# shichaoy/cube_slam

Hardware: AMD Instinct MI355X
Metric: frames/sec front-end (ORB extract + LSD+LBD lines + cuboid: Canny+DT+sweep+score+select) @640x480 (higher is better)
Workload: dtype f64

## Files before the change

cube_slam_amd/csrc/orb.hip:

```cpp
#include "common.h"
#include "orb_quadtree.h"

#include <cfloat>
#include <chrono>
#include <cmath>
#include <omp.h>

namespace {

constexpr int MAXL = 16;
constexpr int HALF_PATCH = 15, PATCH = 31, EDGE_T = 19, MINB = EDGE_T - 3;
constexpr int TW = 64, TH = 16;
constexpr int BLUR_ROWS = 64;

struct Lvl {
    int w, h;
    long off;
    int nCols, nRows, wCell, hCell, maxBX, maxBY;
    int cell_off;
    int tab_x, tab_y;
    float scale; int patch;
};
struct Pyr {
    int nlevels, cells_per_frame, ini_th, min_th;
    long frame_stride;
    int umax[HALF_PATCH + 1];
    int gk[7];
    int tile_off[MAXL + 1], blur_off[MAXL + 1];
    Lvl l[MAXL];
};

__constant__ int c_ring[16][2] = {{0, 3}, {1, 3}, {2, 2}, {3, 1}, {3, 0}, {3, -1}, {2, -2}, {1, -3}, {0, -3}, {-1, -3}, {-2, -2}, {-3, -1}, {-3, 0}, {-3, 1}, {-2, 2}, {-1, 3}};
__device__ const int d_pattern[1024] = {
#include "orb_pattern.inc"
};

#ifndef ORB_RS_ROWS
#define ORB_RS_ROWS 8
#endif
constexpr int RS_ROWS = ORB_RS_ROWS;
__global__ void __launch_bounds__(256) orb_resize(Pyr P, int level, uint8_t *__restrict__ pyr, const int *__restrict__ xofs, const short *__restrict__ ialpha, const int *__restrict__ yofs, const short *__restrict__ ibeta) {
    const Lvl &D = P.l[level], &S = P.l[level - 1];
    const int dx = (blockIdx.x * 64 + (threadIdx.x & 63)) * 4, dy0 = (blockIdx.y * 4 + __builtin_amdgcn_readfirstlane(threadIdx.x >> 6)) * RS_ROWS;
    if (dx >= D.w || dy0 >= D.h) return;
    uint8_t *base = pyr + (long)blockIdx.z * P.frame_stride;
    const uint8_t *src = base + S.off;
    const int nrow = min(RS_ROWS, D.h - dy0);
    int sx[4], a0[4], a1[4];
#pragma unroll
    for (int c = 0; c < 4; c++) {
        const int x = min(dx + c, D.w - 1);
        const int aa = reinterpret_cast<const int *>(ialpha)[D.tab_x + x];
        sx[c] = xofs[D.tab_x + x]; a0[c] = (short)(aa & 0xffff); a1[c] = aa >> 16;
    }
    const bool fast = dx + 3 < D.w && sx[3] - sx[0] <= 4 && sx[0] + 7 < S.w;
    if (fast) {
        uint32_t lo0[RS_ROWS], hi0[RS_ROWS], lo1[RS_ROWS], hi1[RS_ROWS]; int b0[RS_ROWS], b1[RS_ROWS];
#pragma unroll
        for (int r = 0; r < RS_ROWS; r++) {
            const int dy = min(dy0 + r, D.h - 1);
            const int sy = yofs[D.tab_y + dy], sy1 = min(sy + 1, S.h - 1);
            const int bb = reinterpret_cast<const int *>(ibeta)[D.tab_y + dy];
            b0[r] = (short)(bb & 0xffff); b1[r] = bb >> 16;
            const uint8_t *row0 = src + (long)sy * S.w + sx[0], *row1 = src + (long)sy1 * S.w + sx[0];
            lo0[r] = load_u32_unaligned(row0); hi0[r] = load_u32_unaligned(row0 + 4);
            lo1[r] = load_u32_unaligned(row1); hi1[r] = load_u32_unaligned(row1 + 4);
        }
        typedef unsigned short rs_v2u16 __attribute__((ext_vector_type(2)));
        uint32_t sel[4]; rs_v2u16 ap[4];
#pragma unroll
        for (int c = 0; c < 4; c++) { sel[c] = 0x0c010c00u + (uint32_t)(sx[c] - sx[0]) * 0x00010001u; ap[c] = __builtin_bit_cast(rs_v2u16, (uint32_t)a0[c] | ((uint32_t)a1[c] << 16)); }
#pragma unroll
        for (int r = 0; r < RS_ROWS; r++) {
            if (r >= nrow) break;
            uint32_t packed = 0;
#pragma unroll
            for (int c = 0; c < 4; c++) {
                const uint32_t r0 = __builtin_amdgcn_udot2(__builtin_bit_cast(rs_v2u16, __builtin_amdgcn_perm(hi0[r], lo0[r], sel[c])), ap[c], 0u, false);
                const uint32_t r1 = __builtin_amdgcn_udot2(__builtin_bit_cast(rs_v2u16, __builtin_amdgcn_perm(hi1[r], lo1[r], sel[c])), ap[c], 0u, false);
                const uint32_t v = ((__umul24((uint32_t)b0[r], r0 >> 4) >> 16) + (__umul24((uint32_t)b1[r], r1 >> 4) >> 16) + 2u) >> 2;
                packed |= (v & 255u) << (8 * c);
            }
            *reinterpret_cast<cs_u32_unaligned *>(base + D.off + (long)(dy0 + r) * D.w + dx) = packed;
        }
        return;
    }
    for (int r = 0; r < nrow; r++) {
        const int dy = dy0 + r, sy = yofs[D.tab_y + dy], sy1 = min(sy + 1, S.h - 1);
        const int b0 = ibeta[(D.tab_y + dy) * 2], b1 = ibeta[(D.tab_y + dy) * 2 + 1];
        const uint8_t *row0 = src + (long)sy * S.w, *row1 = src + (long)sy1 * S.w;
        for (int c = 0; c < 4 && dx + c < D.w; c++) {
            const int sxc = sx[c], sx1 = min(sxc + 1, S.w - 1);
            const int r0 = row0[sxc] * a0[c] + row0[sx1] * a1[c];
            const int r1 = row1[sxc] * a0[c] + row1[sx1] * a1[c];
            base[D.off + (long)dy * D.w + dx + c] = (uint8_t)((((b0 * (r0 >> 4)) >> 16) + ((b1 * (r1 >> 4)) >> 16) + 2) >> 2);
        }
    }
}

__global__ void __launch_bounds__(256) orb_fast_score(Pyr P, const uint8_t *pyr, uint8_t *smap) {
    int lvq = 0;
    while (lvq + 1 < P.nlevels && (int)blockIdx.x >= P.tile_off[lvq + 1]) lvq++;
    const int lv_u = __builtin_amdgcn_readfirstlane(lvq), tile = (int)blockIdx.x - P.tile_off[lv_u];
    const Lvl &L = P.l[lv_u];
    const int tiles_x = (L.w + TW - 1) / TW;
    const int tx0 = (tile % tiles_x) * TW, ty0 = (tile / tiles_x) * TH;
    __shared__ uint32_t g32[TH + 6][(TW + 8) / 4];
    __shared__ unsigned short s_list[TW * TH];
    __shared__ int s_n;
    uint8_t (*g)[TW + 8] = reinterpret_cast<uint8_t (*)[TW + 8]>(g32);
    const int tq = min(P.ini_th, P.min_th);
    const uint8_t *img = pyr + (long)blockIdx.z * P.frame_stride + L.off;
    if (threadIdx.x == 0) s_n = 0;
    for (int i = threadIdx.x; i < (TH + 6) * ((TW + 8) / 4); i += 256) {
        const int ly = i / ((TW + 8) / 4), k4 = i % ((TW + 8) / 4);
        const int X = tx0 + 4 * k4 - 3, Y = ty0 + ly - 3;
        uint32_t v = 0;
        if (Y >= 0 && Y < L.h) {
            const uint8_t *row = img + (long)Y * L.w;
            if (X >= 0 && X + 3 < L.w) v = load_u32_unaligned(row + X);
            else
                for (int c = 0; c < 4; c++) if (X + c >= 0 && X + c < L.w) v |= (uint32_t)row[X + c] << (8 * c);
        }
        g32[ly][k4] = v;
    }
    __syncthreads();
    const int lx = threadIdx.x & 63, wv = __builtin_amdgcn_readfirstlane((int)(threadIdx.x >> 6));
    static_assert(TH == 16, "four rows per wave");
    unsigned long long cm[4];
    const int x = tx0 + lx;
    const unsigned long long lt = (1ull << lx) - 1;
#pragma unroll
    for (int r = 0; r < 4; r++) {
        const int ly = wv + 4 * r, y = ty0 + ly;
        const int v = g[ly + 3][lx + 3];
        const int d0 = v - (int)g[ly + 6][lx + 3], d4 = v - (int)g[ly + 3][lx + 6], d8 = v - (int)g[ly][lx + 3], d12 = v - (int)g[ly + 3][lx];
        const int dark = max(max(min(d0, d4), min(d4, d8)), max(min(d8, d12), min(d12, d0)));
        const int bright = min(min(max(d0, d4), max(d4, d8)), min(max(d8, d12), max(d12, d0)));
        const bool inb = (unsigned)(x - 3) < (unsigned)(L.w - 6) & (unsigned)(y - 3) < (unsigned)(L.h - 6);
        const bool cand = inb & ((dark > tq) | (bright < -tq));
        if (!cand && x < L.w && y < L.h) smap[(long)blockIdx.z * P.frame_stride + L.off + (long)y * L.w + x] = 0;
        cm[r] = __ballot(cand);
    }
    const int c0 = __popcll(cm[0]), c1 = __popcll(cm[1]), c2 = __popcll(cm[2]), c3 = __popcll(cm[3]);
    if (c0 + c1 + c2 + c3) {
        int base = 0;
        if (lx == 0) base = atomicAdd(&s_n, c0 + c1 + c2 + c3);
        base = __builtin_amdgcn_readfirstlane(base);
        const int off[4] = {base, base + c0, base + c0 + c1, base + c0 + c1 + c2};
#pragma unroll
        for (int r = 0; r < 4; r++)
            if ((cm[r] >> lx) & 1ull) s_list[off[r] + __popcll(cm[r] & lt)] = (unsigned short)((wv + 4 * r) << 8 | lx);
    }
    __syncthreads();
    const int n = s_n;
    for (int i = threadIdx.x; i < n; i += 256) {
        const int ly = s_list[i] >> 8, px = s_list[i] & 255;
        const int v = g[ly + 3][px + 3];
        typedef short v2s __attribute__((ext_vector_type(2)));
        auto swp = [](v2s a) -> v2s { return __builtin_shufflevector(a, a, 1, 0); };
        v2s Pk[8];
#pragma unroll
        for (int k = 0; k < 8; k++) {
            const int ra = g[ly + 3 + c_ring[k][1]][px + 3 + c_ring[k][0]], rb = g[ly + 3 + c_ring[k + 8][1]][px + 3 + c_ring[k + 8][0]];
            v2s r; r.x = (short)(v - ra); r.y = (short)(v - rb);
            Pk[k] = r;
        }
        auto at = [&](const v2s (&X)[8], int k) -> v2s { k &= 15; return k < 8 ? X[k] : swp(X[k - 8]); };
        v2s lo2[8], hi2[8], lo4[8], hi4[8];
#pragma unroll
        for (int k = 0; k < 8; k++) { lo2[k] = __builtin_elementwise_min(Pk[k], at(Pk, k + 1)); hi2[k] = __builtin_elementwise_max(Pk[k], at(Pk, k + 1)); }
#pragma unroll
        for (int k = 0; k < 8; k++) { lo4[k] = __builtin_elementwise_min(lo2[k], at(lo2, k + 2)); hi4[k] = __builtin_elementwise_max(hi2[k], at(hi2, k + 2)); }
        v2s sdp = {-1000, -1000}, sbp = {1000, 1000};
#pragma unroll
        for (int k = 0; k < 8; k++) {
            const v2s lo9 = __builtin_elementwise_min(__builtin_elementwise_min(lo4[k], at(lo4, k + 4)), swp(Pk[k]));
            const v2s hi9 = __builtin_elementwise_max(__builtin_elementwise_max(hi4[k], at(hi4, k + 4)), swp(Pk[k]));
// ... 590 lines not shown
                            }
                            dead[id >> 5] |= 1u << (id & 31);
                        }
                        { int jn = 0; for (int q = 0; q < 4; q++) if (c[q] > 0) { if (c[q] > 1) { if (lane == 0) vn[nvn] = ((unsigned long long)c[q] << 32) | (unsigned)(nn + jn); nvn++; } jn++; } }
                        nn += kk; nfront += kk; cur += kk - 1;
                        __threadfence_block();
                        if (cur >= N) break;
                    }
                    if (cur >= N || cur == ps) fin = true;
                    { unsigned long long *t = vk; vk = vn; vn = t; }
                    nvk = nvn;
                }
                int o = 0;
                if (!ovf) {
                    for (int k0 = nfront - 1; k0 >= 0; k0 -= 64) {
                        const int k = k0 - lane;
                        int id = -1; bool al = false;
                        if (k >= 0) { id = front[k]; al = !((dead[id >> 5] >> (id & 31)) & 1u); }
                        const unsigned long long mm = __ballot(al);
                        if (al) nlist[o + __popcll(mm & ((1ull << lane) - 1))] = (short)id;
                        o += __popcll(mm);
                    }
                    for (int i0 = 0; i0 < n_list; i0 += 64) {
                        const int i = i0 + lane;
                        int id = -1; bool al = false;
                        if (i < n_list) { id = list[i]; al = !((dead[id >> 5] >> (id & 31)) & 1u); }
                        const unsigned long long mm = __ballot(al);
                        if (al) nlist[o + __popcll(mm & ((1ull << lane) - 1))] = (short)id;
                        o += __popcll(mm);
                    }
                }
                if (lane == 0) { s_i[1] = o; s_i[2] = ovf ? 1 : 0; }
            }
            __threadfence_block();
            __syncthreads();
            if (s_i[2]) { overflow = true; break; }
            n_list = s_i[1];
            { short *t = list; list = nlist; nlist = t; }
            finish = true;
        }
    }
    if (overflow) { if (tid == 0) { *status = 1; slot_cnt[fl] = 0; } return; }
    for (int i = tid; i < n_list; i += 256) {
        const int4 nd = nodes[list[i]];
        int best = perm[nd.z];
        float mxr = K[best * 3 + 2];
        for (int p = nd.z + 1; p < nd.w; p++) { const int idx = perm[p]; const float rr = K[idx * 3 + 2]; if (rr > mxr) { best = idx; mxr = rr; } }
        out[i] = SelKP{K[best * 3] + L.minX, K[best * 3 + 1] + L.minY, K[best * 3 + 2], lv, f};
    }
    if (tid == 0) slot_cnt[fl] = n_list;
}
__global__ void __launch_bounds__(256) orb_compact_sel(QtParams Q, const SelKP *slots, const int *slot_cnt, const int *sel_base, SelKP *sel) {
    const int lv = blockIdx.x, f = blockIdx.y, fl = f * Q.nlevels + lv;
    const SelKP *src = slots + (long)f * Q.slots_per_frame + Q.l[lv].slot_off;
    const int n = slot_cnt[fl], b = sel_base[fl];
    for (int i = threadIdx.x; i < n; i += 256) sel[b + i] = src[i];
}

static int qt_half_span(int lo, int hi, int cell, int n_cells, int extent) {
    int s = 0;
    for (int j = 0; j < n_cells; j++) {
        const int a = std::max(lo, 3 + j * cell), b = std::min(hi, std::min(3 + (j + 1) * cell, extent - 3));
        if (b > a) s += (b - a + 1) / 2;
    }
    return s;
}
static long qt_first_split_child_bound(const Lvl &L) {
    const int fw = L.maxBX - MINB, fh = L.maxBY - MINB;
    if (L.nCols < 1 || L.nRows < 1) return 0;
    const int nIni = (int)std::round(static_cast<float>(fw) / fh);
    if (nIni < 1 || nIni > 4) return 0;
    const float hX = static_cast<float>(fw) / nIni;
    const int my = (int)std::ceil(static_cast<float>(fh) / 2);
    const long rows = std::max(qt_half_span(0, my, L.hCell, L.nRows, fh), qt_half_span(my, fh, L.hCell, L.nRows, fh));
    long cols = 0;
    for (int b = 0; b < nIni; b++) {
        const int x0 = (int)(hX * static_cast<float>(b)), x1 = (int)(hX * static_cast<float>(b + 1)), mx = x0 + (int)std::ceil(static_cast<float>(x1 - x0) / 2);
        cols = std::max<long>(cols, qt_half_span(std::max(x0 - 1, 0), mx, L.wCell, L.nCols, fw));
        cols = std::max<long>(cols, qt_half_span(mx, b == nIni - 1 ? fw : x1 + 1, L.wCell, L.nCols, fw));
    }
    return cols * rows;
}

}

struct cs_orb {
    int nfeatures = 0, nlevels = 0, W = 0, H = 0, max_frames = 0, n_frames = 0;
    float scaleFactor = 0;
    std::vector<float> mvScaleFactor, mvInvScaleFactor, mvLevelSigma2, mvInvLevelSigma2;
    std::vector<int> mnFeaturesPerLevel;
    Pyr P{};
    int max_tiles = 0, max_blur_blocks = 0;
    long cand_cap = 0, cand_alloc = 0;
    uint8_t *d_pyr = nullptr, *d_smap = nullptr, *d_blur = nullptr;
    unsigned long long *d_cell_mask = nullptr;
    int *d_xofs = nullptr, *d_yofs = nullptr, *d_cell_count = nullptr, *d_cell_base = nullptr, *d_level_total = nullptr, *d_level_base = nullptr;
    short *d_ialpha = nullptr, *d_ibeta = nullptr;
    float *d_cand = nullptr, *d_angle = nullptr;
    SelKP *d_sel = nullptr;
    QtParams Q{}; bool gpu_quadtree = false; size_t qt_lds = 0;
    int *d_qperm = nullptr, *d_qtmp = nullptr, *d_slot_cnt = nullptr, *d_sel_base = nullptr, *d_qstatus = nullptr; int4 *d_qnodes = nullptr; SelKP *d_slots = nullptr;
    std::vector<int> sel_base;
    bool cand_valid = false;
    cs_keypoint *d_kps = nullptr;
    unsigned long long *d_desc = nullptr;
    long sel_cap = 0;
    std::vector<int> level_base;
    std::vector<cs_orb_host::Cand> cand;
    std::vector<SelKP> sel;
    std::vector<int> frame_first;
};

int cs_orb_device_frame(const cs_orb *e, int frame, const cs_keypoint **d_kps, const unsigned long long **d_desc, int *n) {
    if (!e || frame < 0 || frame >= e->n_frames || (int)e->frame_first.size() <= frame + 1) return CS_ERR_BAD_ARG;
    const int b0 = e->frame_first[frame];
    *d_kps = e->d_kps + b0; *d_desc = e->d_desc + (size_t)b0 * 4; *n = e->frame_first[frame + 1] - b0;
    return CS_OK;
}

int cs_orb_device_pyramid(const cs_orb *e, cs_orb_pyramid_view *out) {
    static_assert(CS_ORB_MAX_LEVELS == MAXL, "cs_orb_pyramid_view holds every level");
    if (!e || !out) return CS_ERR_BAD_ARG;
    out->d_pyr = e->d_pyr; out->frame_stride = e->P.frame_stride; out->nlevels = e->nlevels; out->n_frames = e->n_frames; out->W = e->W; out->H = e->H;
    out->scale_factor = e->scaleFactor;
    for (int l = 0; l < e->nlevels; l++) {
        out->off[l] = e->P.l[l].off; out->w[l] = e->P.l[l].w; out->h[l] = e->P.l[l].h;
        out->scale[l] = e->mvScaleFactor[l]; out->inv_scale[l] = e->mvInvScaleFactor[l];
    }
    return CS_OK;
}

extern "C" {

void cs_orb_destroy(cs_ctx *ctx, cs_orb *e) {
    if (!e) return;
    if (ctx) { hipSetDevice(ctx->device); hipStreamSynchronize(ctx->stream); }
    void *ptrs[] = {e->d_cell_mask, e->d_pyr, e->d_smap, e->d_blur, e->d_xofs, e->d_yofs, e->d_cell_count, e->d_cell_base, e->d_level_total, e->d_level_base,
                    e->d_ialpha, e->d_ibeta, e->d_cand, e->d_angle, e->d_sel, e->d_kps, e->d_desc, e->d_qperm, e->d_qtmp, e->d_slot_cnt, e->d_sel_base, e->d_qstatus,
                    e->d_qnodes, e->d_slots};
    for (void *p : ptrs) cs_dfree(ctx, p);
    delete e;
}

int cs_orb_create(cs_ctx *ctx, int nfeatures, float scaleFactor, int nlevels, int iniThFAST, int minThFAST, int width, int height,
                  int max_frames, cs_orb **out) {
    if (!ctx || !out || nfeatures < 1 || nlevels < 1 || nlevels > MAXL || !(scaleFactor > 1.0f) || width < 64 || height < 64 || max_frames < 1 ||
        iniThFAST < 0 || iniThFAST > 255 || minThFAST < 0 || minThFAST > 255)
        return CS_ERR_BAD_ARG;
    *out = nullptr;
    CS_HIP(ctx, hipSetDevice(ctx->device));
    cs_orb *e = new (std::nothrow) cs_orb();
    if (!e) return CS_ERR_NOMEM;
    e->nfeatures = nfeatures; e->nlevels = nlevels; e->W = width; e->H = height; e->max_frames = max_frames; e->scaleFactor = scaleFactor;
    e->mvScaleFactor.resize(nlevels); e->mvLevelSigma2.resize(nlevels); e->mvInvScaleFactor.resize(nlevels); e->mvInvLevelSigma2.resize(nlevels);
    e->mvScaleFactor[0] = 1.0f; e->mvLevelSigma2[0] = 1.0f;
    for (int i = 1; i < nlevels; i++) { e->mvScaleFactor[i] = e->mvScaleFactor[i - 1] * scaleFactor; e->mvLevelSigma2[i] = e->mvScaleFactor[i] * e->mvScaleFactor[i]; }
    for (int i = 0; i < nlevels; i++) { e->mvInvScaleFactor[i] = 1.0f / e->mvScaleFactor[i]; e->mvInvLevelSigma2[i] = 1.0f / e->mvLevelSigma2[i]; }
    e->mnFeaturesPerLevel.resize(nlevels);
    {
        float factor = 1.0f / scaleFactor;
        float nDesired = nfeatures * (1 - factor) / (1 - (float)std::pow((double)factor, (double)nlevels));
        int sum = 0;
        for (int level = 0; level < nlevels - 1; level++) { e->mnFeaturesPerLevel[level] = h_cvRound(nDesired); sum += e->mnFeaturesPerLevel[level]; nDesired *= factor; }
        e->mnFeaturesPerLevel[nlevels - 1] = std::max(nfeatures - sum, 0);
    }
    Pyr &P = e->P;
    P.nlevels = nlevels; P.ini_th = iniThFAST; P.min_th = minThFAST;
    {
        int v, v0, vmax = h_cvFloor(HALF_PATCH * std::sqrt(2.f) / 2 + 1), vmin = h_cvCeil(HALF_PATCH * std::sqrt(2.f) / 2);
        const double hp2 = HALF_PATCH * HALF_PATCH;
        for (v = 0; v <= vmax; ++v) P.umax[v] = h_cvRound(std::sqrt(hp2 - v * v));
        for (v = HALF_PATCH, v0 = 0; v >= vmin; --v) { while (P.umax[v0] == P.umax[v0 + 1]) ++v0; P.umax[v] = v0; ++v0; }
    }
    {
        float cf[7];
        double scale2X = -0.5 / (2.0 * 2.0), sum = 0;
        for (int i = 0; i < 7; i++) { double x = i - 3.0; cf[i] = (float)std::exp(scale2X * x * x); sum += cf[i]; }
        sum = 1. / sum;
        for (int i = 0; i < 7; i++) { cf[i] = (float)(cf[i] * sum); P.gk[i] = h_cvRound(cf[i] * 256.f); }
    }
    std::vector<int> xofs, yofs;
    std::vector<short> ialpha, ibeta;
    long off = 0;
    int cells = 0;
    e->max_tiles = 0;
    long cand_per_frame = 0;
    auto sat_short = [](float v) { int i = h_cvRound(v); return (short)(i < -32768 ? -32768 : (i > 32767 ? 32767 : i)); };
    for (int l = 0; l < nlevels; l++) {
        Lvl &L = P.l[l];
        float scale = e->mvInvScaleFactor[l];
        L.w = h_cvRound((float)width * scale); L.h = h_cvRound((float)height * scale);
        L.off = off; off += ((long)L.w * L.h + 63) / 64 * 64;
        L.maxBX = L.w - EDGE_T + 3; L.maxBY = L.h - EDGE_T + 3;
        const float fw = (float)(L.maxBX - MINB), fh = (float)(L.maxBY - MINB);
        L.nCols = (int)(fw / 30.f); L.nRows = (int)(fh / 30.f);
        if (L.nCols < 1 || L.nRows < 1) { L.nCols = L.nRows = 0; L.wCell = L.hCell = 1; }
        else { L.wCell = (int)std::ceil(fw / L.nCols); L.hCell = (int)std::ceil(fh / L.nRows); }
        if (L.wCell > 58 || L.hCell > 58) { delete e; return CS_ERR_CAPACITY; }
        L.cell_off = cells; cells += L.nCols * L.nRows;
        L.scale = e->mvScaleFactor[l]; L.patch = (int)(PATCH * e->mvScaleFactor[l]);
        L.tab_x = (int)xofs.size(); L.tab_y = (int)yofs.size();
        if (l > 0) {
            const int sw = P.l[l - 1].w, sh = P.l[l - 1].h;
            const double scale_x = 1. / ((double)L.w / sw), scale_y = 1. / ((double)L.h / sh);
            for (int dx = 0; dx < L.w; dx++) {
                float fx = (float)((dx + 0.5) * scale_x - 0.5);
                int sx = h_cvFloor(fx);
                fx -= sx;
                if (sx < 0) { fx = 0; sx = 0; }
                if (sx >= sw - 1) { fx = 0; sx = sw - 1; }
                xofs.push_back(sx); ialpha.push_back(sat_short((1.f - fx) * 2048)); ialpha.push_back(sat_short(fx * 2048));
            }
            for (int dy = 0; dy < L.h; dy++) {
                float fy = (float)((dy + 0.5) * scale_y - 0.5);
                int sy = h_cvFloor(fy);
                fy -= sy;
                if (sy < 0) { fy = 0; sy = 0; }
                if (sy >= sh - 1) { fy = 0; sy = sh - 1; }
                yofs.push_back(sy); ibeta.push_back(sat_short((1.f - fy) * 2048)); ibeta.push_back(sat_short(fy * 2048));
            }
        }
        e->max_tiles = std::max(e->max_tiles, ((L.w + TW - 1) / TW) * ((L.h + TH - 1) / TH));
        e->max_blur_blocks = std::max(e->max_blur_blocks, ((L.w + 255) / 256) * ((L.h + BLUR_ROWS - 1) / BLUR_ROWS));
        P.tile_off[l + 1] = P.tile_off[l] + ((L.w + TW - 1) / TW) * ((L.h + TH - 1) / TH);
        P.blur_off[l + 1] = P.blur_off[l] + ((L.w + 255) / 256) * ((L.h + BLUR_ROWS - 1) / BLUR_ROWS);
        cand_per_frame += (long)((L.w + 1) / 2) * ((L.h + 1) / 2);
    }
    P.frame_stride = off; P.cells_per_frame = cells;
    e->cand_cap = cand_per_frame * max_frames;
    e->sel_cap = (long)(nfeatures + 4 * nlevels + 64) * max_frames * 2;
#define A_(call) do { int r__ = (call); if (r__ != CS_OK) { cs_orb_destroy(ctx, e); return r__; } } while (0)
    A_(cs_dalloc(ctx, &e->d_pyr, (size_t)off * max_frames));
    A_(cs_dalloc(ctx, &e->d_smap, (size_t)off * max_frames));
    A_(cs_dalloc(ctx, &e->d_blur, (size_t)off * max_frames));
    A_(cs_dalloc(ctx, &e->d_xofs, xofs.size()));
    A_(cs_dalloc(ctx, &e->d_yofs, yofs.size()));
    A_(cs_dalloc(ctx, &e->d_ialpha, ialpha.size()));
    A_(cs_dalloc(ctx, &e->d_ibeta, ibeta.size()));
    A_(cs_dalloc(ctx, &e->d_cell_count, (size_t)cells * max_frames));
    A_(cs_dalloc(ctx, &e->d_cell_mask, (size_t)cells * max_frames * CELL_MASK_WORDS));
    A_(cs_dalloc(ctx, &e->d_cell_base, (size_t)cells * max_frames));
    A_(cs_dalloc(ctx, &e->d_level_total, (size_t)nlevels * max_frames));
    A_(cs_dalloc(ctx, &e->d_level_base, (size_t)nlevels * max_frames + 1));
    A_(cs_dalloc(ctx, &e->d_sel, (size_t)e->sel_cap));
    A_(cs_dalloc(ctx, &e->d_angle, (size_t)e->sel_cap));
    A_(cs_dalloc(ctx, &e->d_kps, (size_t)e->sel_cap));
    A_(cs_dalloc(ctx, &e->d_desc, (size_t)e->sel_cap * 4));
    {
        QtParams &Q = e->Q;
        Q.nlevels = nlevels;
        int node_off = 0, slot_off = 0, maxN = 0;
        bool ok = true;
        for (int l = 0; l < nlevels; l++) {
            const Lvl &L = e->P.l[l];
            QtLevel &q = Q.l[l];
            q.N = e->mnFeaturesPerLevel[l]; q.minX = MINB; q.maxX = L.maxBX; q.minY = MINB; q.maxY = L.maxBY;
            q.capn = 12 * std::max(q.N, 1) + 64; q.node_off = node_off; q.slot_off = slot_off;
            node_off += q.capn; slot_off += 4 * std::max(q.N, 1) + 16;
            maxN = std::max(maxN, q.N);
            if (L.maxBX >= 32768 || L.maxBY >= 32768) ok = false;
            if (qt_first_split_child_bound(L) >= 65536) ok = false;
        }
        Q.nodes_per_frame = node_off; Q.slots_per_frame = slot_off;
        const int CAPL = 4 * std::max(maxN, 1) + 16, CAPV = std::max(maxN, 1) + 8, CAPN = 12 * std::max(maxN, 1) + 64;
        e->qt_lds = (size_t)8 * CAPL + (size_t)8 * CAPV * 3 + (size_t)4 * (CAPV + 1) * 2 + (size_t)4 * ((CAPN + 31) / 32) + (size_t)2 * CAPV + 64;
        const char *force = getenv("CUBESLAM_ORB_QUADTREE");
        e->gpu_quadtree = ok && maxN >= 1 && CAPN < 32768 && e->qt_lds <= 150 * 1024 && !(force && !strcmp(force, "host"));
        if (e->gpu_quadtree) {
            A_(cs_dalloc(ctx, &e->d_qnodes, (size_t)Q.nodes_per_frame * max_frames)); A_(cs_dalloc(ctx, &e->d_slots, (size_t)Q.slots_per_frame * max_frames));
            A_(cs_dalloc(ctx, &e->d_slot_cnt, (size_t)nlevels * max_frames)); A_(cs_dalloc(ctx, &e->d_sel_base, (size_t)nlevels * max_frames + 1));
            A_(cs_dalloc(ctx, &e->d_qstatus, (size_t)1));
        }
    }
    A_(cs_h2d(ctx, e->d_xofs, xofs.data(), xofs.size()));
    A_(cs_h2d(ctx, e->d_yofs, yofs.data(), yofs.size()));
    A_(cs_h2d(ctx, e->d_ialpha, ialpha.data(), ialpha.size()));
    A_(cs_h2d(ctx, e->d_ibeta, ibeta.data(), ibeta.size()));
    { hipError_t er = hipStreamSynchronize(ctx->stream); if (er != hipSuccess) { ctx->err = hipGetErrorString(er); cs_orb_destroy(ctx, e); return CS_ERR_HIP; } }
#undef A_
    *out = e;
    return CS_OK;
}

int cs_orb_get_table(const cs_orb *e, int which, void *out) {
    if (!e || !out) return CS_ERR_BAD_ARG;
    const std::vector<float> *t = which == 0 ? &e->mvScaleFactor : which == 1 ? &e->mvInvScaleFactor : which == 2 ? &e->mvLevelSigma2 : which == 3 ? &e->mvInvLevelSigma2 : nullptr;
    if (t) { memcpy(out, t->data(), t->size() * sizeof(float)); return CS_OK; }
    if (which == 4) { memcpy(out, e->mnFeaturesPerLevel.data(), e->mnFeaturesPerLevel.size() * sizeof(int)); return CS_OK; }
    return CS_ERR_BAD_ARG;
}

int cs_orb_upload(cs_ctx *ctx, cs_orb *e, const uint8_t *gray, int n_frames, int stride) {
    if (!ctx || !e || !gray || n_frames < 1 || n_frames > e->max_frames || stride < e->W) return CS_ERR_BAD_ARG;
    CS_HIP(ctx, hipSetDevice(ctx->device));
    e->n_frames = n_frames;
    for (int f = 0; f < n_frames; f++)
        CS_HIP(ctx, hipMemcpy2DAsync(e->d_pyr + (long)f * e->P.frame_stride, (size_t)e->W, gray + (size_t)f * stride * e->H, (size_t)stride, (size_t)e->W,
                                     (size_t)e->H, hipMemcpyHostToDevice, ctx->stream));
    CS_HIP(ctx, hipStreamSynchronize(ctx->stream));
    return CS_OK;
}

int cs_orb_geometry(const cs_orb *e, int *width, int *height, int *max_frames) {
    if (!e) return CS_ERR_BAD_ARG;
    *width = e->W; *height = e->H; *max_frames = e->max_frames;
    return CS_OK;
}
int cs_orb_set_frames_device(cs_ctx *ctx, cs_orb *e, const uint8_t *d_gray, int n_frames) {
    if (!ctx || !e || !d_gray || n_frames < 1 || n_frames > e->max_frames) return CS_ERR_BAD_ARG;
    CS_HIP(ctx, hipSetDevice(ctx->device));
    e->n_frames = n_frames;
    const size_t fb = (size_t)e->W * e->H;
    CS_HIP(ctx, hipMemcpy2DAsync(e->d_pyr, (size_t)e->P.frame_stride, d_gray, fb, fb, (size_t)n_frames, hipMemcpyDeviceToDevice, ctx->stream));
    return CS_OK;
}

int cs_orb_run(cs_ctx *ctx, cs_orb *e) {
    if (!ctx || !e || e->n_frames < 1) return CS_ERR_BAD_ARG;
    CS_HIP(ctx, hipSetDevice(ctx->device));
    const Pyr &P = e->P;
    const int F = e->n_frames, NL = P.nlevels;
    for (int l = 1; l < NL; l++) {
        CS_LAUNCH(ctx, "orb_resize", orb_resize, dim3((P.l[l].w + 255) / 256, (P.l[l].h + 4 * RS_ROWS - 1) / (4 * RS_ROWS), F), dim3(256), 0, P, l, e->d_pyr, e->d_xofs, e->d_ialpha,
                  e->d_yofs, e->d_ibeta);
    }
    CS_LAUNCH(ctx, "orb_fast_score", orb_fast_score, dim3(P.tile_off[NL], 1, F), dim3(256), 0, P, e->d_pyr, e->d_smap);
    CS_LAUNCH(ctx, "orb_cells", orb_cells, dim3((P.cells_per_frame + CELLS_PER_WG - 1) / CELLS_PER_WG, F), dim3(64 * CELLS_PER_WG), 0, P, e->d_smap, 0, e->d_cell_count, e->d_cell_base, e->d_cand, e->d_cell_mask);
    CS_LAUNCH(ctx, "orb_scan", orb_scan_cells, dim3(NL, F), dim3(64), 0, P, e->d_cell_count, e->d_cell_base, e->d_level_total);
    CS_LAUNCH(ctx, "orb_scan", orb_scan_levels, dim3(1), dim3(64), 0, F * NL, e->d_level_total, e->d_level_base);
    CS_LAUNCH(ctx, "orb_scan", orb_rebase_cells, dim3((F * P.cells_per_frame + 255) / 256), dim3(256), 0, P, F, e->d_level_base, e->d_cell_base);
    e->level_base.resize((size_t)F * NL + 1);
    int r = cs_d2h(ctx, e->level_base.data(), e->d_level_base, e->level_base.size()); if (r) return r;
    CS_HIP(ctx, hipStreamSynchronize(ctx->stream));
    const long total = e->level_base[(size_t)F * NL];
    if (total > e->cand_cap) { ctx->err = "ORB candidate capacity exceeded"; return CS_ERR_CAPACITY; }
    if (total > e->cand_alloc) {
        void *old[] = {e->d_cand, e->d_qperm, e->d_qtmp};
        for (void *q : old) cs_dfree(ctx, q);
        e->d_cand = nullptr; e->d_qperm = nullptr; e->d_qtmp = nullptr; e->cand_alloc = 0;
        const long cap = std::min<long>(e->cand_cap, total + total / 4 + 4096);
        r = cs_dalloc(ctx, &e->d_cand, (size_t)cap * 3); if (r) return r;
        if (e->gpu_quadtree) { r = cs_dalloc(ctx, &e->d_qperm, (size_t)cap); if (r) return r; r = cs_dalloc(ctx, &e->d_qtmp, (size_t)cap); if (r) return r; }
        e->cand_alloc = cap;
    }
    CS_LAUNCH(ctx, "orb_cells", orb_cells, dim3((P.cells_per_frame + CELLS_PER_WG - 1) / CELLS_PER_WG, F), dim3(64 * CELLS_PER_WG), 0, P, e->d_smap, 1, e->d_cell_count, e->d_cell_base, e->d_cand, e->d_cell_mask);
    bool on_device = e->gpu_quadtree;
    if (on_device) {
        CS_HIP(ctx, hipMemsetAsync(e->d_qstatus, 0, sizeof(int), ctx->stream));
        if (e->qt_lds > 64 * 1024) CS_HIP(ctx, hipFuncSetAttribute((const void *)orb_quadtree, hipFuncAttributeMaxDynamicSharedMemorySize, (int)e->qt_lds));
        CS_LAUNCH(ctx, "orb_quadtree", orb_quadtree, dim3(F, NL), dim3(256), e->qt_lds, e->Q, e->d_level_base, e->d_cand, e->d_qperm, e->d_qtmp, e->d_qnodes, e->d_slots,
                  e->d_slot_cnt, e->d_qstatus);
        CS_LAUNCH(ctx, "orb_scan", orb_scan_levels, dim3(1), dim3(64), 0, F * NL, e->d_slot_cnt, e->d_sel_base);
        e->sel_base.resize((size_t)F * NL + 1);
        int qstatus = 0;
        r = cs_d2h(ctx, e->sel_base.data(), e->d_sel_base, e->sel_base.size()); if (r) return r;
        r = cs_d2h(ctx, &qstatus, e->d_qstatus, 1); if (r) return r;
        CS_LAUNCH(ctx, "orb_blur", orb_blur, dim3(P.blur_off[NL], 1, F), dim3(64), 0, P, e->d_pyr, e->d_blur);
        CS_HIP(ctx, hipStreamSynchronize(ctx->stream));
        e->cand_valid = false;
        if (qstatus != 0) on_device = false;
        else {
            const int n = e->sel_base[(size_t)F * NL];
            e->frame_first.assign((size_t)F + 1, 0);
            for (int f = 0; f <= F; f++) e->frame_first[f] = e->sel_base[(size_t)std::min(f, F) * NL];
            if (n > e->sel_cap) { ctx->err = "ORB keypoint capacity exceeded"; return CS_ERR_CAPACITY; }
            if (n == 0) return CS_OK;
            CS_LAUNCH(ctx, "orb_compact_sel", orb_compact_sel, dim3(NL, F), dim3(256), 0, e->Q, e->d_slots, e->d_slot_cnt, e->d_sel_base, e->d_sel);
            CS_LAUNCH(ctx, "orb_angle", orb_angle, dim3((n + 7) / 8), dim3(256), 0, P, e->d_pyr, e->d_sel, n, e->d_angle);
            CS_LAUNCH(ctx, "orb_desc", orb_desc, dim3((n + 3) / 4), dim3(256), 0, P, e->d_blur, e->d_sel, e->d_angle, n, e->d_kps, e->d_desc);
            CS_HIP(ctx, hipGetLastError());
            return CS_OK;
        }
    }
    const bool blur_done = e->gpu_quadtree;
    e->cand.resize((size_t)std::max<long>(total, 1));
    r = cs_d2h(ctx, (float *)e->cand.data(), e->d_cand, (size_t)total * 3); if (r) return r;
    hipEvent_t ev_cand = ctx->get_event();
    CS_HIP(ctx, hipEventRecord(ev_cand, ctx->stream));
    if (!blur_done) CS_LAUNCH(ctx, "orb_blur", orb_blur, dim3(P.blur_off[NL], 1, F), dim3(64), 0, P, e->d_pyr, e->d_blur);
    CS_HIP(ctx, hipEventSynchronize(ev_cand));
    e->cand_valid = true;
    ctx->pool.push_back(ev_cand);
    const auto t_host0 = std::chrono::steady_clock::now();
    e->sel.clear();
    e->frame_first.assign((size_t)F + 1, 0);
    {
        std::vector<std::vector<SelKP>> per((size_t)F * NL);
    cs_omp_prepare();
#pragma omp parallel num_threads(std::max(1, std::min(ctx->host_threads, F * NL / 4)))
        {
            cs_orb_host::QuadTree qt;
            std::vector<int> idx;
#pragma omp for schedule(dynamic, 1)
            for (int fl = 0; fl < F * NL; fl++) {
                const int f = fl / NL, l = fl % NL;
                const Lvl &L = P.l[l];
                const long b0 = e->level_base[fl], n = e->level_base[fl + 1] - b0;
                if (n <= 0 || L.nCols == 0) continue;
                const cs_orb_host::Cand *K = e->cand.data() + b0;
                qt.distribute(K, (int)n, MINB, L.maxBX, MINB, L.maxBY, e->mnFeaturesPerLevel[l], idx);
                std::vector<SelKP> &o = per[fl];
                o.reserve(idx.size());
                for (int id : idx) o.push_back(SelKP{K[id].x + MINB, K[id].y + MINB, K[id].response, l, f});
            }
        }
        for (int f = 0; f < F; f++) {
            e->frame_first[f] = (int)e->sel.size();
            for (int l = 0; l < NL; l++) e->sel.insert(e->sel.end(), per[(size_t)f * NL + l].begin(), per[(size_t)f * NL + l].end());
// ... 100 lines not shown
```

Measured before the change: 28220.

## Fuse ORB pyramid levels into one tiled LDS kernel with precomputed plans

Replaces the per-level resize launches with a fused orb_pyramid kernel. Each workgroup loads a source tile plus halo into LDS and computes several successive pyramid levels from LDS, ping-ponging between two buffers. A host-side planner chooses tile sizes and level segments under an LDS budget, precomputes per-tile offset and weight tables, and checks coverage. This is meant to remove the chain of dependent launches and the global-memory round trips between levels, at the cost of redundant halo computation, LDS pressure and a more complex plan.

```diff
diff --git a/cube_slam_amd/csrc/orb.hip b/cube_slam_amd/csrc/orb.hip
--- a/cube_slam_amd/csrc/orb.hip
+++ b/cube_slam_amd/csrc/orb.hip
@@ -35,65 +35,129 @@
 #include "orb_pattern.inc"
 };
 
-#ifndef ORB_RS_ROWS
-#define ORB_RS_ROWS 8
-#endif
-constexpr int RS_ROWS = ORB_RS_ROWS;
-__global__ void __launch_bounds__(256) orb_resize(Pyr P, int level, uint8_t *__restrict__ pyr, const int *__restrict__ xofs, const short *__restrict__ ialpha, const int *__restrict__ yofs, const short *__restrict__ ibeta) {
-    const Lvl &D = P.l[level], &S = P.l[level - 1];
-    const int dx = (blockIdx.x * 64 + (threadIdx.x & 63)) * 4, dy0 = (blockIdx.y * 4 + __builtin_amdgcn_readfirstlane(threadIdx.x >> 6)) * RS_ROWS;
-    if (dx >= D.w || dy0 >= D.h) return;
+struct PyrTile {
+    int nx0, ny0, nw, nh;
+    int ox0, oy0, ox1, oy1;
+    int pitch;
+    int ytab, xtab;
+    int pad;
+};
+struct PyrSeg { int lo, hi, ntiles, plan_off, lds, buf1; long tab_off; int tab_bytes; };
+constexpr int PYR_ROWS = 4;
+constexpr int PYR_LDS_BUDGET = 40 * 1024;
+typedef uint32_t pyr_u32x2 __attribute__((ext_vector_type(2), aligned(1)));
+typedef uint32_t pyr_u32x4 __attribute__((ext_vector_type(4), aligned(1)));
+typedef uint32_t pyr_u32x4a __attribute__((ext_vector_type(4)));
+
+__global__ void __launch_bounds__(256) __attribute__((amdgpu_waves_per_eu(8))) orb_pyramid(Pyr P, int lo, int hi, const PyrTile *__restrict__ plan, const uint8_t *__restrict__ tabs, int tab_bytes,
+                                                                                               int buf1, int tab_lds, uint8_t *__restrict__ pyr) {
+    extern __shared__ __attribute__((aligned(16))) uint8_t py_lds[];
+    const int tid = threadIdx.x;
+    const PyrTile *T = plan + (size_t)blockIdx.x * (hi - lo + 1);
+    if (T[0].nw <= 0 || T[0].nh <= 0) return;
     uint8_t *base = pyr + (long)blockIdx.z * P.frame_stride;
-    const uint8_t *src = base + S.off;
-    const int nrow = min(RS_ROWS, D.h - dy0);
-    int sx[4], a0[4], a1[4];
-#pragma unroll
-    for (int c = 0; c < 4; c++) {
-        const int x = min(dx + c, D.w - 1);
-        const int aa = reinterpret_cast<const int *>(ialpha)[D.tab_x + x];
-        sx[c] = xofs[D.tab_x + x]; a0[c] = (short)(aa & 0xffff); a1[c] = aa >> 16;
-    }
-    const bool fast = dx + 3 < D.w && sx[3] - sx[0] <= 4 && sx[0] + 7 < S.w;
-    if (fast) {
-        uint32_t lo0[RS_ROWS], hi0[RS_ROWS], lo1[RS_ROWS], hi1[RS_ROWS]; int b0[RS_ROWS], b1[RS_ROWS];
-#pragma unroll
-        for (int r = 0; r < RS_ROWS; r++) {
-            const int dy = min(dy0 + r, D.h - 1);
-            const int sy = yofs[D.tab_y + dy], sy1 = min(sy + 1, S.h - 1);
-            const int bb = reinterpret_cast<const int *>(ibeta)[D.tab_y + dy];
-            b0[r] = (short)(bb & 0xffff); b1[r] = bb >> 16;
-            const uint8_t *row0 = src + (long)sy * S.w + sx[0], *row1 = src + (long)sy1 * S.w + sx[0];
-            lo0[r] = load_u32_unaligned(row0); hi0[r] = load_u32_unaligned(row0 + 4);
-            lo1[r] = load_u32_unaligned(row1); hi1[r] = load_u32_unaligned(row1 + 4);
-        }
-        typedef unsigned short rs_v2u16 __attribute__((ext_vector_type(2)));
-        uint32_t sel[4]; rs_v2u16 ap[4];
-#pragma unroll
-        for (int c = 0; c < 4; c++) { sel[c] = 0x0c010c00u + (uint32_t)(sx[c] - sx[0]) * 0x00010001u; ap[c] = __builtin_bit_cast(rs_v2u16, (uint32_t)a0[c] | ((uint32_t)a1[c] << 16)); }
-#pragma unroll
-        for (int r = 0; r < RS_ROWS; r++) {
-            if (r >= nrow) break;
-            uint32_t packed = 0;
-#pragma unroll
-            for (int c = 0; c < 4; c++) {
-                const uint32_t r0 = __builtin_amdgcn_udot2(__builtin_bit_cast(rs_v2u16, __builtin_amdgcn_perm(hi0[r], lo0[r], sel[c])), ap[c], 0u, false);
-                const uint32_t r1 = __builtin_amdgcn_udot2(__builtin_bit_cast(rs_v2u16, __builtin_amdgcn_perm(hi1[r], lo1[r], sel[c])), ap[c], 0u, false);
-                const uint32_t v = ((__umul24((uint32_t)b0[r], r0 >> 4) >> 16) + (__umul24((uint32_t)b1[r], r1 >> 4) >> 16) + 2u) >> 2;
-                packed |= (v & 255u) << (8 * c);
-            }
-            *reinterpret_cast<cs_u32_unaligned *>(base + D.off + (long)(dy0 + r) * D.w + dx) = packed;
-        }
-        return;
-    }
-    for (int r = 0; r < nrow; r++) {
-        const int dy = dy0 + r, sy = yofs[D.tab_y + dy], sy1 = min(sy + 1, S.h - 1);
-        const int b0 = ibeta[(D.tab_y + dy) * 2], b1 = ibeta[(D.tab_y + dy) * 2 + 1];
-        const uint8_t *row0 = src + (long)sy * S.w, *row1 = src + (long)sy1 * S.w;
-        for (int c = 0; c < 4 && dx + c < D.w; c++) {
-            const int sxc = sx[c], sx1 = min(sxc + 1, S.w - 1);
-            const int r0 = row0[sxc] * a0[c] + row0[sx1] * a1[c];
-            const int r1 = row1[sxc] * a0[c] + row1[sx1] * a1[c];
-            base[D.off + (long)dy * D.w + dx + c] = (uint8_t)((((b0 * (r0 >> 4)) >> 16) + ((b1 * (r1 >> 4)) >> 16) + 2) >> 2);
+    {
+        const pyr_u32x4a *g = reinterpret_cast<const pyr_u32x4a *>(tabs + (size_t)blockIdx.x * tab_bytes);
+        pyr_u32x4a *t = reinterpret_cast<pyr_u32x4a *>(py_lds + tab_lds);
+        const int n = tab_bytes >> 4;
+        for (int i = tid; i < n; i += 4 * 256) {
+            pyr_u32x4a v[4];
+#pragma unroll
+            for (int k = 0; k < 4; k++) v[k] = g[min(i + 256 * k, n - 1)];
+#pragma unroll
+            for (int k = 0; k < 4; k++)
+                if (i + 256 * k < n) t[i + 256 * k] = v[k];
+        }
+    }
+    {
+        const PyrTile &S = T[0];
+        const int sw = P.l[lo].w, cpr = S.pitch >> 4, rpp = 256 / cpr, r0 = tid / cpr, c = tid - r0 * cpr;
+        const uint8_t *g = base + P.l[lo].off + (long)S.ny0 * sw + S.nx0 + 16 * c;
+        for (int r = r0 < rpp ? r0 : S.nh; r < S.nh; r += 4 * rpp) {
+            pyr_u32x4 v[4];
+#pragma unroll
+            for (int k = 0; k < 4; k++) v[k] = *reinterpret_cast<const pyr_u32x4 *>(g + (long)min(r + k * rpp, S.nh - 1) * sw);
+#pragma unroll
+            for (int k = 0; k < 4; k++)
+                if (r + k * rpp < S.nh) *reinterpret_cast<pyr_u32x4a *>(py_lds + (r + k * rpp) * S.pitch + 16 * c) = v[k];
+        }
+    }
+    typedef unsigned short rs_v2u16 __attribute__((ext_vector_type(2)));
+    for (int l = lo + 1; l <= hi; l++) {
+        const PyrTile D = T[l - lo];
+        const int lw = P.l[l].w;
+        if (D.nw <= 0 || D.nh <= 0) break;
+        const uint8_t *src = py_lds + (((l - lo - 1) & 1) ? buf1 : 0);
+        uint8_t *dst = py_lds + (((l - lo) & 1) ? buf1 : 0);
+        const int2 *yt = reinterpret_cast<const int2 *>(py_lds + D.ytab);
+        const bool keep = l < hi;
+        const int ncg = (D.nw + 3) >> 2, nstripe = 256 / ncg, stripe = tid / ncg, cg = tid - stripe * ncg, rps = (D.nh + nstripe - 1) / nstripe;
+        const int y_begin = stripe * rps, y_end = stripe < nstripe ? min(D.nh, y_begin + rps) : 0;
+        __syncthreads();
+        const pyr_u32x4a sx4 = *reinterpret_cast<const pyr_u32x4a *>(py_lds + D.xtab + 32 * cg), ap4 = *reinterpret_cast<const pyr_u32x4a *>(py_lds + D.xtab + 32 * cg + 16);
+        const int sx[4] = {(int)sx4.x, (int)sx4.y, (int)sx4.z, (int)sx4.w};
+        const uint32_t ap[4] = {ap4.x, ap4.y, ap4.z, ap4.w};
+        const bool fast = sx[3] - sx[0] <= 6;
+        uint32_t sel[4];
+#pragma unroll
+        for (int c = 0; c < 4; c++) sel[c] = 0x0c010c00u + (uint32_t)(sx[c] - sx[0]) * 0x00010001u;
+        const int gx = D.nx0 + 4 * cg;
+        const bool own_x = gx >= D.ox0 && gx < D.ox1, whole = gx + 3 < D.ox1;
+        const int own_lo = own_x ? D.oy0 - D.ny0 : 0, own_hi = own_x ? D.oy1 - D.ny0 : 0;
+        uint8_t *out = base + P.l[l].off + (long)D.ny0 * lw + gx;
+        uint8_t *keep_at = dst + 4 * cg;
+        const auto put = [&](int yy, uint32_t packed) {
+            if (keep) *reinterpret_cast<uint32_t *>(keep_at + yy * D.pitch) = packed;
+            if (yy >= own_lo && yy < own_hi) {
+                uint8_t *o = out + (long)yy * lw;
+                if (whole) *reinterpret_cast<cs_u32_unaligned *>(o) = packed;
+                else {
+#pragma unroll
+                    for (int c = 0; c < 3; c++)
+                        if (gx + c < D.ox1) o[c] = (uint8_t)(packed >> (8 * c));
+                }
+            }
+        };
+        if (fast) {
+            for (int y = y_begin; y < y_end; y += PYR_ROWS) {
+                int2 t[PYR_ROWS]; pyr_u32x2 w0[PYR_ROWS], w1[PYR_ROWS];
+#pragma unroll
+                for (int r = 0; r < PYR_ROWS; r++) t[r] = yt[min(y + r, y_end - 1)];
+#pragma unroll
+                for (int r = 0; r < PYR_ROWS; r++) {
+                    w0[r] = *reinterpret_cast<const pyr_u32x2 *>(src + (t[r].x & 0xffff) + sx[0]);
+                    w1[r] = *reinterpret_cast<const pyr_u32x2 *>(src + ((uint32_t)t[r].x >> 16) + sx[0]);
+                }
+#pragma unroll
+                for (int r = 0; r < PYR_ROWS; r++) {
+                    if (y + r >= y_end) break;
+                    const uint32_t b0 = (uint32_t)t[r].y & 0xffffu, b1 = (uint32_t)t[r].y >> 16;
+                    uint32_t packed = 0;
+#pragma unroll
+                    for (int c = 0; c < 4; c++) {
+                        const uint32_t r0 = __builtin_amdgcn_udot2(__builtin_bit_cast(rs_v2u16, __builtin_amdgcn_perm(w0[r].y, w0[r].x, sel[c])), __builtin_bit_cast(rs_v2u16, ap[c]), 0u, false);
+                        const uint32_t r1 = __builtin_amdgcn_udot2(__builtin_bit_cast(rs_v2u16, __builtin_amdgcn_perm(w1[r].y, w1[r].x, sel[c])), __builtin_bit_cast(rs_v2u16, ap[c]), 0u, false);
+                        const uint32_t v = ((__umul24(b0, r0 >> 4) >> 16) + (__umul24(b1, r1 >> 4) >> 16) + 2u) >> 2;
+                        packed |= (v & 255u) << (8 * c);
+                    }
+                    put(y + r, packed);
+                }
+            }
+        } else {
+            for (int y = y_begin; y < y_end; y++) {
+                const int2 t = yt[y];
+                const uint8_t *row0 = src + (t.x & 0xffff), *row1 = src + ((uint32_t)t.x >> 16);
+                const uint32_t b0 = (uint32_t)t.y & 0xffffu, b1 = (uint32_t)t.y >> 16;
+                uint32_t packed = 0;
+#pragma unroll
+                for (int c = 0; c < 4; c++) {
+                    const uint32_t a0 = ap[c] & 0xffffu, a1 = ap[c] >> 16;
+                    const uint32_t r0 = row0[sx[c]] * a0 + row0[sx[c] + 1] * a1, r1 = row1[sx[c]] * a0 + row1[sx[c] + 1] * a1;
+                    const uint32_t v = ((__umul24(b0, r0 >> 4) >> 16) + (__umul24(b1, r1 >> 4) >> 16) + 2u) >> 2;
+                    packed |= (v & 255u) << (8 * c);
+                }
+                put(y, packed);
+            }
         }
     }
 }
@@ -850,6 +914,131 @@
     return cols * rows;
 }
 
+struct PyrTables { std::vector<int> xofs, yofs; std::vector<short> ialpha, ibeta; };
+static bool pyr_plan_segment(const Pyr &P, const PyrTables &tb, int lo, int hi, int tw, int th, std::vector<PyrTile> &out, std::vector<uint8_t> &tabs, PyrSeg &seg, double *overhead) {
+    const std::vector<int> &xofs = tb.xofs, &yofs = tb.yofs;
+    const int nl = hi - lo + 1, TX = (P.l[lo].w + tw - 1) / tw, TY = (P.l[lo].h + th - 1) / th;
+    out.assign((size_t)TX * TY * nl, PyrTile{});
+    int buf[2] = {0, 0}, tab_max = 0;
+    double computed = 0, owned = 0;
+    for (int ty = 0; ty < TY; ty++)
+        for (int tx = 0; tx < TX; tx++) {
+            PyrTile *T = &out[((size_t)ty * TX + tx) * nl];
+            for (int l = lo; l <= hi; l++) {
+                const Lvl &L = P.l[l];
+                PyrTile &t = T[l - lo];
+                t.ox0 = tx == 0 ? 0 : (int)((long)tx * L.w / TX) & ~3; t.ox1 = tx == TX - 1 ? L.w : (int)((long)(tx + 1) * L.w / TX) & ~3;
+                t.oy0 = (int)((long)ty * L.h / TY); t.oy1 = (int)((long)(ty + 1) * L.h / TY);
+            }
+            int tab = 0;
+            for (int l = hi; l >= lo; l--) {
+                PyrTile &t = T[l - lo];
+                int x0 = t.ox0, x1 = t.ox1, y0 = t.oy0, y1 = t.oy1;
+                if (x1 <= x0 || y1 <= y0) x0 = x1 = y0 = y1 = 0;
+                if (l < hi && T[l - lo + 1].nw > 0 && T[l - lo + 1].nh > 0) {
+                    const PyrTile &u = T[l - lo + 1];
+                    const Lvl &U = P.l[l + 1], &L = P.l[l];
+                    const int fx0 = xofs[U.tab_x + u.nx0], fx1 = std::min(xofs[U.tab_x + u.nx0 + u.nw - 1] + 1, L.w - 1) + 1;
+                    const int fy0 = yofs[U.tab_y + u.ny0], fy1 = std::min(yofs[U.tab_y + u.ny0 + u.nh - 1] + 1, L.h - 1) + 1;
+                    if (x1 <= x0) { x0 = fx0; x1 = fx1; y0 = fy0; y1 = fy1; }
+                    else { x0 = std::min(x0, fx0); x1 = std::max(x1, fx1); y0 = std::min(y0, fy0); y1 = std::max(y1, fy1); }
+                }
+                x0 &= ~3;
+                t.nx0 = x0; t.ny0 = y0; t.nw = x1 - x0; t.nh = y1 - y0;
+                t.pitch = l == lo ? (t.nw + 15) / 16 * 16 : (t.nw + 3) / 4 * 4;
+                if (t.nw > 1024) return false;
+                buf[(l - lo) & 1] = std::max(buf[(l - lo) & 1], t.pitch * t.nh + 16);
+                if (l > lo) { t.ytab = tab; tab += (8 * t.nh + 15) / 16 * 16; t.xtab = tab; tab += 32 * ((t.nw + 3) / 4); computed += (double)t.nw * t.nh; owned += (double)std::max(t.ox1 - t.ox0, 0) * std::max(t.oy1 - t.oy0, 0); }
+            }
+            tab_max = std::max(tab_max, tab);
+        }
+    buf[0] = (buf[0] + 15) / 16 * 16; buf[1] = (buf[1] + 15) / 16 * 16;
+    if (buf[0] >= 65536 || buf[1] >= 65536 || buf[0] + buf[1] + tab_max > PYR_LDS_BUDGET) return false;
+    seg.lo = lo; seg.hi = hi; seg.ntiles = TX * TY; seg.lds = buf[0] + buf[1] + tab_max; seg.buf1 = buf[0]; seg.tab_bytes = tab_max;
+    tabs.assign((size_t)seg.ntiles * tab_max, 0);
+    for (int t = 0; t < seg.ntiles; t++) {
+        uint32_t *img = reinterpret_cast<uint32_t *>(tabs.data() + (size_t)t * tab_max);
+        for (int l = lo + 1; l <= hi; l++) {
+            PyrTile &d = out[(size_t)t * nl + (l - lo)];
+            const PyrTile &s = out[(size_t)t * nl + (l - lo - 1)];
+            const Lvl &L = P.l[l], &S = P.l[l - 1];
+            for (int i = 0; i < d.nh; i++) {
+                const int sy = yofs[L.tab_y + d.ny0 + i], sy1 = std::min(sy + 1, S.h - 1);
+                img[d.ytab / 4 + 2 * i] = (uint32_t)((sy - s.ny0) * s.pitch) | ((uint32_t)((sy1 - s.ny0) * s.pitch) << 16);
+                img[d.ytab / 4 + 2 * i + 1] = (uint16_t)tb.ibeta[2 * (L.tab_y + d.ny0 + i)] | ((uint32_t)(uint16_t)tb.ibeta[2 * (L.tab_y + d.ny0 + i) + 1] << 16);
+            }
+            for (int i = 0; i < (d.nw + 3) / 4 * 4; i++) {
+                const int x = L.tab_x + d.nx0 + std::min(i, d.nw - 1);
+                img[d.xtab / 4 + (i / 4) * 8 + (i & 3)] = (uint32_t)(xofs[x] - s.nx0);
+                img[d.xtab / 4 + (i / 4) * 8 + 4 + (i & 3)] = (uint16_t)tb.ialpha[2 * x] | ((uint32_t)(uint16_t)tb.ialpha[2 * x + 1] << 16);
+            }
+            d.ytab += buf[0] + buf[1]; d.xtab += buf[0] + buf[1];
+        }
+    }
+    *overhead = owned > 0 ? computed / owned : 1.0;
+    return true;
+}
+
+static bool pyr_plan_check(const Pyr &P, const PyrTables &tb, const PyrSeg &seg, const PyrTile *plan) {
+    const std::vector<int> &xofs = tb.xofs, &yofs = tb.yofs;
+    const int nl = seg.hi - seg.lo + 1;
+    for (int l = seg.lo + 1; l <= seg.hi; l++) {
+        const Lvl &L = P.l[l], &S = P.l[l - 1];
+        std::vector<uint8_t> cover((size_t)L.w * L.h, 0);
+        for (int t = 0; t < seg.ntiles; t++) {
+            const PyrTile &d = plan[(size_t)t * nl + (l - seg.lo)], &s = plan[(size_t)t * nl + (l - seg.lo - 1)];
+            const bool own = d.ox1 > d.ox0 && d.oy1 > d.oy0;
+            if (own) {
+                if (d.ox0 < 0 || d.oy0 < 0 || d.ox1 > L.w || d.oy1 > L.h || (d.ox0 & 3)) return false;
+                if (d.ox0 < d.nx0 || d.oy0 < d.ny0 || d.ox1 > d.nx0 + d.nw || d.oy1 > d.ny0 + d.nh) return false;
+                for (int y = d.oy0; y < d.oy1; y++)
+                    for (int x = d.ox0; x < d.ox1; x++)
+                        if (cover[(size_t)y * L.w + x]++) return false;
+            }
+            if (d.nw <= 0 || d.nh <= 0) { if (own) return false; continue; }
+            if ((d.nx0 & 3) || d.nx0 < 0 || d.ny0 < 0 || d.nx0 + d.nw > L.w || d.ny0 + d.nh > L.h || d.pitch < d.nw || (d.pitch & 3)) return false;
+            if (s.nx0 < 0 || s.ny0 < 0 || s.nx0 + s.nw > S.w || s.ny0 + s.nh > S.h || s.pitch < s.nw || (l - 1 == seg.lo && (s.pitch & 15))) return false;
+            for (int x = d.nx0; x < d.nx0 + d.nw; x++) {
+                const int sx = xofs[L.tab_x + x], sx1 = std::min(sx + 1, S.w - 1);
+                if (sx < s.nx0 || sx1 >= s.nx0 + s.nw) return false;
+            }
+            for (int y = d.ny0; y < d.ny0 + d.nh; y++) {
+                const int sy = yofs[L.tab_y + y], sy1 = std::min(sy + 1, S.h - 1);
+                if (sy < s.ny0 || sy1 >= s.ny0 + s.nh) return false;
+            }
+        }
+        for (uint8_t c : cover)
+            if (c != 1) return false;
+    }
+    return true;
+}
+
+static bool pyr_plan_build(const Pyr &P, const PyrTables &tb, std::vector<PyrSeg> &segs, std::vector<PyrTile> &plan, std::vector<uint8_t> &tabs) {
+    static const int sizes[][2] = {{128, 96}, {112, 96}, {96, 64}, {64, 48}, {32, 32}, {16, 16}, {8, 8}, {4, 4}};
+    segs.clear(); plan.clear(); tabs.clear();
+    for (int lo = 0; lo + 1 < P.nlevels;) {
+        bool found = false;
+        std::vector<PyrTile> tiles;
+        std::vector<uint8_t> seg_tabs;
+        PyrSeg seg{};
+        for (int hi = P.nlevels - 1; hi > lo && !found; hi--)
+            for (const auto &sz : sizes) {
+                double overhead = 0;
+                if (!pyr_plan_segment(P, tb, lo, hi, sz[0], sz[1], tiles, seg_tabs, seg, &overhead)) continue;
+                found = overhead <= 2.0 || hi == lo + 1;
+                break;
+            }
+        if (!found) return false;
+        seg.plan_off = (int)plan.size(); seg.tab_off = (long)tabs.size();
+        plan.insert(plan.end(), tiles.begin(), tiles.end());
+        tabs.insert(tabs.end(), seg_tabs.begin(), seg_tabs.end());
+        if (!pyr_plan_check(P, tb, seg, plan.data() + seg.plan_off)) return false;
+        segs.push_back(seg);
+        lo = seg.hi;
+    }
+    return true;
+}
+
 }
 
 struct cs_orb {
@@ -862,8 +1051,8 @@
     long cand_cap = 0, cand_alloc = 0;
     uint8_t *d_pyr = nullptr, *d_smap = nullptr, *d_blur = nullptr;
     unsigned long long *d_cell_mask = nullptr;
-    int *d_xofs = nullptr, *d_yofs = nullptr, *d_cell_count = nullptr, *d_cell_base = nullptr, *d_level_total = nullptr, *d_level_base = nullptr;
-    short *d_ialpha = nullptr, *d_ibeta = nullptr;
+    int *d_cell_count = nullptr, *d_cell_base = nullptr, *d_level_total = nullptr, *d_level_base = nullptr;
+    PyrTile *d_pyr_plan = nullptr; uint8_t *d_pyr_tabs = nullptr; std::vector<PyrSeg> pyr_segs;
     float *d_cand = nullptr, *d_angle = nullptr;
     SelKP *d_sel = nullptr;
     QtParams Q{}; bool gpu_quadtree = false; size_t qt_lds = 0;
@@ -903,8 +1092,8 @@
 void cs_orb_destroy(cs_ctx *ctx, cs_orb *e) {
     if (!e) return;
     if (ctx) { hipSetDevice(ctx->device); hipStreamSynchronize(ctx->stream); }
-    void *ptrs[] = {e->d_cell_mask, e->d_pyr, e->d_smap, e->d_blur, e->d_xofs, e->d_yofs, e->d_cell_count, e->d_cell_base, e->d_level_total, e->d_level_base,
-                    e->d_ialpha, e->d_ibeta, e->d_cand, e->d_angle, e->d_sel, e->d_kps, e->d_desc, e->d_qperm, e->d_qtmp, e->d_slot_cnt, e->d_sel_base, e->d_qstatus,
+    void *ptrs[] = {e->d_cell_mask, e->d_pyr, e->d_smap, e->d_blur, e->d_cell_count, e->d_cell_base, e->d_level_total, e->d_level_base,
+                    e->d_pyr_plan, e->d_pyr_tabs, e->d_cand, e->d_angle, e->d_sel, e->d_kps, e->d_desc, e->d_qperm, e->d_qtmp, e->d_slot_cnt, e->d_sel_base, e->d_qstatus,
                     e->d_qnodes, e->d_slots};
     for (void *p : ptrs) cs_dfree(ctx, p);
     delete e;
@@ -947,8 +1136,9 @@
         sum = 1. / sum;
         for (int i = 0; i < 7; i++) { cf[i] = (float)(cf[i] * sum); P.gk[i] = h_cvRound(cf[i] * 256.f); }
     }
-    std::vector<int> xofs, yofs;
-    std::vector<short> ialpha, ibeta;
+    PyrTables tb;
+    std::vector<int> &xofs = tb.xofs, &yofs = tb.yofs;
+    std::vector<short> &ialpha = tb.ialpha, &ibeta = tb.ibeta;
     long off = 0;
     int cells = 0;
     e->max_tiles = 0;
@@ -996,15 +1186,16 @@
     }
     P.frame_stride = off; P.cells_per_frame = cells;
     e->cand_cap = cand_per_frame * max_frames;
+    std::vector<PyrTile> pyr_plan;
+    std::vector<uint8_t> pyr_tabs;
+    if (!pyr_plan_build(P, tb, e->pyr_segs, pyr_plan, pyr_tabs)) { ctx->err = "ORB pyramid: no tile plan fits the kernel, or the plan failed its check"; delete e; return CS_ERR_CAPACITY; }
     e->sel_cap = (long)(nfeatures + 4 * nlevels + 64) * max_frames * 2;
 #define A_(call) do { int r__ = (call); if (r__ != CS_OK) { cs_orb_destroy(ctx, e); return r__; } } while (0)
     A_(cs_dalloc(ctx, &e->d_pyr, (size_t)off * max_frames));
     A_(cs_dalloc(ctx, &e->d_smap, (size_t)off * max_frames));
     A_(cs_dalloc(ctx, &e->d_blur, (size_t)off * max_frames));
-    A_(cs_dalloc(ctx, &e->d_xofs, xofs.size()));
-    A_(cs_dalloc(ctx, &e->d_yofs, yofs.size()));
-    A_(cs_dalloc(ctx, &e->d_ialpha, ialpha.size()));
-    A_(cs_dalloc(ctx, &e->d_ibeta, ibeta.size()));
+    A_(cs_dalloc(ctx, &e->d_pyr_plan, pyr_plan.size()));
+    A_(cs_dalloc(ctx, &e->d_pyr_tabs, pyr_tabs.size()));
     A_(cs_dalloc(ctx, &e->d_cell_count, (size_t)cells * max_frames));
     A_(cs_dalloc(ctx, &e->d_cell_mask, (size_t)cells * max_frames * CELL_MASK_WORDS));
     A_(cs_dalloc(ctx, &e->d_cell_base, (size_t)cells * max_frames));
@@ -1040,10 +1231,8 @@
             A_(cs_dalloc(ctx, &e->d_qstatus, (size_t)1));
         }
     }
-    A_(cs_h2d(ctx, e->d_xofs, xofs.data(), xofs.size()));
-    A_(cs_h2d(ctx, e->d_yofs, yofs.data(), yofs.size()));
-    A_(cs_h2d(ctx, e->d_ialpha, ialpha.data(), ialpha.size()));
-    A_(cs_h2d(ctx, e->d_ibeta, ibeta.data(), ibeta.size()));
+    A_(cs_h2d(ctx, e->d_pyr_plan, pyr_plan.data(), pyr_plan.size()));
+    A_(cs_h2d(ctx, e->d_pyr_tabs, pyr_tabs.data(), pyr_tabs.size()));
     { hipError_t er = hipStreamSynchronize(ctx->stream); if (er != hipSuccess) { ctx->err = hipGetErrorString(er); cs_orb_destroy(ctx, e); return CS_ERR_HIP; } }
 #undef A_
     *out = e;
@@ -1088,10 +1277,10 @@
     CS_HIP(ctx, hipSetDevice(ctx->device));
     const Pyr &P = e->P;
     const int F = e->n_frames, NL = P.nlevels;
-    for (int l = 1; l < NL; l++) {
-        CS_LAUNCH(ctx, "orb_resize", orb_resize, dim3((P.l[l].w + 255) / 256, (P.l[l].h + 4 * RS_ROWS - 1) / (4 * RS_ROWS), F), dim3(256), 0, P, l, e->d_pyr, e->d_xofs, e->d_ialpha,
-                  e->d_yofs, e->d_ibeta);
-    }
+    for (const PyrSeg &s : e->pyr_segs)
+        if (s.ntiles > 0)
+            CS_LAUNCH(ctx, "orb_resize", orb_pyramid, dim3(s.ntiles, 1, F), dim3(256), (size_t)s.lds, P, s.lo, s.hi, e->d_pyr_plan + s.plan_off, e->d_pyr_tabs + s.tab_off, s.tab_bytes, s.buf1,
+                      s.lds - s.tab_bytes, e->d_pyr);
     CS_LAUNCH(ctx, "orb_fast_score", orb_fast_score, dim3(P.tile_off[NL], 1, F), dim3(256), 0, P, e->d_pyr, e->d_smap);
     CS_LAUNCH(ctx, "orb_cells", orb_cells, dim3((P.cells_per_frame + CELLS_PER_WG - 1) / CELLS_PER_WG, F), dim3(64 * CELLS_PER_WG), 0, P, e->d_smap, 0, e->d_cell_count, e->d_cell_base, e->d_cand, e->d_cell_mask);
     CS_LAUNCH(ctx, "orb_scan", orb_scan_cells, dim3(NL, F), dim3(64), 0, P, e->d_cell_count, e->d_cell_base, e->d_level_total);
```

New measurement: 28450 (median of 2 runs). No clear change (+0.8%).
